# nirvanesque/headCT_foundation

Hardware: AMD Instinct MI355X
Metric: CT-volumes/sec MAE pretrain step (96^3, ViT-B/16^3, mask 0.75) (higher is better)
Workload: dtype bf16; 1 GPU; BASELINE config #2: MAE ViT-B/16^3, 96^3x1ch, mask 0.75, full train step (fwd+bwd+clip+AdamW+LR); per_gpu_batch=256, global_batch=256, parallelism=dp1, init=reference init, seed 42

## Files before the change

headct_foundation_amd/_lib.py:

```python
from __future__ import annotations

import ctypes as C
import os
from typing import Optional

HERE = os.path.dirname(os.path.abspath(__file__))
LIB_PATH = os.path.join(HERE, "libheadct_hip.so")

HCT_F32, HCT_BF16, HCT_F16 = 0, 1, 2
NORM_LAYERNORM, NORM_RMSNORM = 0, 1
HCT_ACT_NONE, HCT_ACT_GELU, HCT_ACT_DGELU, HCT_ACT_TANH, HCT_ACT_GELU_D, HCT_ACT_MULAUX = 0, 1, 2, 3, 4, 5
ACT_NONE, ACT_GELU, ACT_DGELU = 0, 1, 2

c_void_p, c_int, c_float, c_size_t, c_int64 = C.c_void_p, C.c_int, C.c_float, C.c_size_t, C.c_int64


class GemmArgs(C.Structure):
    _fields_ = [
        ("M", c_int), ("N", c_int), ("K", c_int),
        ("A", c_void_p), ("a_dtype", c_int), ("lda", c_int64), ("transA", c_int),
        ("B", c_void_p), ("b_dtype", c_int), ("ldb", c_int64), ("transB", c_int),
        ("C", c_void_p), ("c_dtype", c_int), ("ldc", c_int64),
        ("bias", c_void_p), ("residual", c_void_p), ("ldr", c_int64),
        ("act", c_int),
# ... 4 lines not shown


class GemmPlanInfo(C.Structure):
    _fields_ = [("kernel", c_int), ("epilogue_mode", c_int), ("fuse_colsum", c_int), ("row_tiles_per_wave", c_int), ("tiles", c_int),
                ("grid", c_int), ("sk_tiles", c_int), ("sk_wgs", c_int), ("splits", c_int), ("r_chunk", c_int), ("colsum_bytes", c_size_t),
                ("stream_k_offset", c_size_t), ("slab_bytes", c_size_t), ("workspace_bytes", c_size_t), ("walk_width", c_int)]


class ProfShape(C.Structure):
    _fields_ = [("M", c_int), ("N", c_int), ("K", c_int), ("mode", c_int), ("tiles", c_int), ("sk_tiles", c_int),
                ("launches", c_int64), ("total_ms", C.c_double), ("work", C.c_double), ("bytes", C.c_double)]


def prof_shapes(lib, kernel_class: int, cap: int = 256):
    buf = (ProfShape * cap)()
    n = lib.hct_prof_shapes(kernel_class, C.cast(buf, c_void_p), cap)
    if n < 0:
        raise HctError("hct_prof_shapes failed")
    return [buf[i] for i in range(min(n, cap))]


class MaeConfig(C.Structure):
    _fields_ = [
        ("input_size", c_int), ("patch_size", c_int), ("in_chans", c_int), ("mask_ratio", C.c_double),
        ("pos_embed", c_int),
        ("encoder_depth", c_int), ("encoder_embed_dim", c_int), ("encoder_mlp_dim", c_int), ("encoder_num_heads", c_int),
        ("decoder_depth", c_int), ("decoder_embed_dim", c_int), ("decoder_mlp_dim", c_int), ("decoder_num_heads", c_int),
        ("norm_pix_loss", c_int), ("use_bias", c_int),
        ("encoder_only", c_int), ("num_register_tokens", c_int), ("final_norm_eps", c_float),
        ("lora_rank", c_int),
        ("norm_kind", c_int),
        ("dropout_rate", c_float),
        ("drop_path_rate", c_float),
        ("patch_dropout", C.c_double),
    ]


class ParamInfo(C.Structure):
    _fields_ = [
        ("name", C.c_char * 96), ("ndim", c_int), ("shape", c_int64 * 5), ("offset", c_int64), ("numel", c_int64),
        ("requires_grad", c_int), ("is_matrix", c_int), ("bf16_t_offset", c_int64),
    ]


_PROTOS = {
    "hct_last_error_string": (C.c_char_p, []),
    "hct_version": (c_int, []),
    "hct_has_mfma_kernels": (c_int, []),
    "hct_gemm_workspace_bytes": (c_size_t, [C.POINTER(GemmArgs)]),
    "hct_gemm_nt_flags_offset": (c_size_t, [c_size_t]),
    "hct_gemm_describe": (c_int, [C.POINTER(GemmArgs), c_int, c_size_t, C.POINTER(GemmPlanInfo)]),
    "hct_gemm_stream_k_items": (c_int, [c_int, c_int, c_int, c_int, C.POINTER(C.c_uint32), C.POINTER(C.c_uint32)]),
    "hct_gemm_nt_walk": (c_int, [c_int, c_int, c_int, c_int, C.POINTER(c_int)]),
    "hct_set_cu_reserve": (None, [c_int]),
    "hct_gemm": (c_int, [C.POINTER(GemmArgs), c_void_p, c_size_t, c_void_p]),
    "hct_mask_rank": (c_int, [c_void_p, c_int, c_int, c_int, c_void_p, c_void_p, c_void_p, c_void_p]),
    "hct_patch_gather": (c_int, [c_void_p, c_int, c_void_p, c_int, c_int, c_int, c_int, c_int, c_int, c_void_p, c_int, c_void_p]),
    "hct_encoder_assemble_fwd": (c_int, [c_void_p, c_int, c_void_p, c_void_p, c_void_p, c_int, c_int, c_int, c_int, c_void_p, c_void_p]),
    "hct_encoder_assemble_bwd": (c_int, [c_void_p, c_void_p, c_int, c_int, c_int, c_int, c_void_p, c_int, c_void_p, c_void_p, c_void_p, c_size_t, c_void_p]),
    "hct_assemble_bwd_workspace_bytes": (c_size_t, [c_int]),
    "hct_layernorm_fwd": (c_int, [c_void_p, c_void_p, c_void_p, c_int, c_int, c_float, c_void_p, c_int, c_void_p, c_void_p, c_void_p]),
    "hct_layernorm_bwd_workspace_bytes": (c_size_t, [c_int, c_int]),
    "hct_layernorm_bwd": (c_int, [c_void_p, c_int, c_void_p, c_void_p, c_void_p, c_void_p, c_void_p, c_int, c_int, c_void_p, c_void_p,
                                  c_int, c_void_p, c_void_p, c_void_p, c_void_p, c_size_t, c_void_p]),
    "hct_layernorm_bwd_mapped": (c_int, [c_void_p, c_int, c_void_p, c_void_p, c_void_p, c_void_p, c_void_p, c_void_p, c_int, c_int, c_void_p,
                                         c_void_p, c_int, c_void_p, c_void_p, c_void_p, c_void_p, c_size_t, c_void_p]),
    "hct_rmsnorm_fwd": (c_int, [c_void_p, c_void_p, c_int, c_int, c_float, c_void_p, c_int, c_void_p, c_void_p]),
    "hct_rmsnorm_bwd_workspace_bytes": (c_size_t, [c_int, c_int]),
    "hct_rmsnorm_bwd": (c_int, [c_void_p, c_int, c_void_p, c_void_p, c_void_p, c_void_p, c_int, c_int, c_void_p, c_void_p, c_int, c_void_p,
                                c_void_p, c_void_p, c_size_t, c_void_p]),
    "hct_rmsnorm_bwd_mapped": (c_int, [c_void_p, c_int, c_void_p, c_void_p, c_void_p, c_void_p, c_void_p, c_int, c_int, c_void_p, c_void_p,
                                       c_int, c_void_p, c_void_p, c_void_p, c_size_t, c_void_p]),
    "hct_tail_rows": (c_int, [c_void_p, c_int, c_int, c_int, c_void_p, c_void_p, c_void_p]),
    "hct_gather_rows": (c_int, [c_void_p, c_void_p, c_int, c_int, c_void_p, c_void_p]),
    "hct_attention_fwd": (c_int, [c_void_p, c_int, c_int, c_int, c_int, c_int, c_void_p, c_void_p, c_void_p]),
    "hct_attention_bwd": (c_int, [c_void_p, c_void_p, c_void_p, c_void_p, c_int, c_int, c_int, c_int, c_int, c_void_p, c_void_p]),
    "hct_debug_force_simple_attention": (None, [c_int]),
    "hct_dropout_mask": (c_int, [C.c_uint64, c_int, c_int, c_int64, c_int, c_int, c_float, c_void_p, c_void_p]),
    "hct_dropout_apply": (c_int, [c_void_p, c_int, c_void_p, c_int, c_void_p, c_void_p, c_void_p, c_int64, c_int64, c_int64, c_int64, C.c_uint64,
                                  c_int, c_float, c_void_p]),
    "hct_attention_dropout_fwd": (c_int, [c_void_p, c_int, c_int, c_int, c_int, c_int, c_float, C.c_uint64, c_int, c_void_p, c_void_p, c_void_p]),
    "hct_attention_dropout_bwd": (c_int, [c_void_p, c_void_p, c_void_p, c_void_p, c_int, c_int, c_int, c_int, c_int, c_float, C.c_uint64, c_int,
                                          c_void_p, c_void_p]),
    "hct_drop_path_scales": (c_int, [C.c_uint64, C.POINTER(c_int), C.POINTER(c_float), c_int, c_int, c_void_p, c_void_p]),
    "hct_residual_drop_apply": (c_int, [c_void_p, c_int, c_void_p, c_int, c_void_p, c_int64, c_int64, c_void_p, C.c_uint64, c_int, c_float,
                                        c_void_p]),
    "hct_mae_plan_set_dropout": (c_int, [c_void_p, c_int, C.c_uint64]),
    "hct_decoder_assemble_fwd": (c_int, [c_void_p, c_int, c_void_p, c_void_p, c_void_p, c_void_p, c_int, c_int, c_int, c_int, c_void_p, c_void_p]),
    "hct_decoder_assemble_bwd": (c_int, [c_void_p, c_void_p, c_void_p, c_int, c_int, c_int, c_int, c_void_p, c_int, c_void_p, c_void_p,
                                         c_void_p, c_size_t, c_void_p]),
    "hct_masked_mse": (c_int, [c_void_p, c_int, c_void_p, c_int, c_void_p, c_int, c_int, c_int, c_int, c_int, c_float, c_void_p, c_void_p, c_void_p, c_void_p, c_void_p]),
    "hct_unpatchify": (c_int, [c_void_p, c_int, c_int, c_int, c_int, c_int, c_int, c_void_p, c_void_p]),
    "hct_vit_assemble_fwd": (c_int, [c_void_p, c_int, c_void_p, c_void_p, c_void_p, c_int, c_int, c_int, c_int, c_void_p, c_void_p]),
    "hct_channel_norm": (c_int, [c_void_p, c_void_p, c_void_p, c_float, c_void_p, c_int, c_int64, c_int, c_void_p]),
    "hct_query_attention": (c_int, [c_void_p, c_int, c_void_p, c_int, c_int, c_int, c_int, c_int, c_float, c_void_p, c_void_p]),
    "hct_head_linear": (c_int, [c_void_p, c_int64, c_int, c_void_p, c_void_p, c_float, c_void_p, c_void_p, c_int, c_void_p, c_int, c_int,
                                c_int, c_void_p]),
    "hct_batchnorm_stats": (c_int, [c_void_p, c_int, c_int, c_float, c_void_p, c_void_p, c_void_p, c_void_p, c_void_p]),
    "hct_softmax_xent": (c_int, [c_void_p, c_void_p, c_int, c_int, c_void_p, c_void_p, c_void_p, c_void_p]),
    "hct_sigmoid_bce_workspace_bytes": (c_size_t, [c_int, c_int]),
    "hct_sigmoid_bce": (c_int, [c_void_p, c_void_p, c_void_p, c_int, c_int, c_void_p, c_void_p, c_void_p, c_void_p, c_void_p, c_size_t, c_void_p]),
    "hct_mix_volumes": (c_int, [c_void_p, c_int, c_int, c_int, c_void_p, c_void_p, c_void_p]),
    "hct_mix_xent": (c_int, [c_void_p, c_void_p, c_void_p, c_float, c_int, c_int, c_void_p, c_void_p, c_void_p, c_void_p]),
    "hct_head_linear_wgrad": (c_int, [c_void_p, c_void_p, c_void_p, c_float, c_void_p, c_int, c_int, c_int, c_void_p, c_void_p, c_void_p]),
    "hct_bn_rows_workspace_bytes": (c_size_t, [c_int, c_int]),
    "hct_bn_stats_rows": (c_int, [c_void_p, c_int, c_int64, c_int, c_int, c_float, c_void_p, c_void_p, c_void_p, c_void_p, c_void_p,
# ... 207 lines not shown
```

headct_foundation_amd/csrc/gemm.hip:

```cpp
#include "common.h"
#include "gemm_plan.h"
#include "prof.h"

#include <cstdlib>
#include <cstring>
#include <vector>

namespace hct {

struct Epilogue {
  const float* bias;
  const float* residual;
  int64_t ldr;
  int act;
  void* aux; int aux_dtype; int64_t ldaux;
  void* C; int c_dtype; int64_t ldc;
  void* C2; int c2_dtype; int64_t ldc2;
  float alpha;
  float* colsum_partial;
  int aux_deriv;
};

__device__ __forceinline__ void store4(void* base, int dtype, int64_t off, f32x4 v) {
  if (dtype == HCT_BF16) Vec4<bf16>::store((bf16*)base + off, v);
// ... 218 lines not shown
    const int c = wave * 4 + i;
    const int row = c * 8 + (lane >> 3);
    const int src_chunk = (lane & 7) ^ ((row >> 1) & 7);
    voa[i] = (uint32_t)(row * lda * 2 + src_chunk * 16);
    vob[i] = (uint32_t)(row * ldb * 2 + src_chunk * 16);
  }
  auto stage = [&](int buf, int k0) {
    unsigned char* base = smem + buf * 32768;
#pragma unroll
    for (int i = 0; i < 4; ++i) {
      const int c = wave * 4 + i;
      __builtin_amdgcn_raw_ptr_buffer_load_lds(ra, (lds_void*)(base + c * 1024), 16, voa[i] + k0 * 2, 0, 0, 0);
      __builtin_amdgcn_raw_ptr_buffer_load_lds(rb, (lds_void*)(base + 16384 + c * 1024), 16, vob[i] + k0 * 2, 0, 0, 0);
    }
  };

  const int wr = wave >> 1, wc = wave & 1;
  const int frow = lane & 15, fchk = lane >> 4, swz = (lane >> 1) & 7;
  f32x4 acc[4][4];
#pragma unroll
  for (int i = 0; i < 4; ++i)
#pragma unroll
    for (int j = 0; j < 4; ++j) acc[i][j] = f32x4{0, 0, 0, 0};

  const int nk = K >> 6;
  stage(0, 0);
  __syncthreads();
  for (int kt = 0; kt < nk; ++kt) {
    const int buf = kt & 1;
    if (kt + 1 < nk) stage(buf ^ 1, (kt + 1) << 6);
    const unsigned char* sa = smem + buf * 32768 + (wr * 64 + frow) * 128;
    const unsigned char* sb = smem + buf * 32768 + 16384 + (wc * 64 + frow) * 128;
#pragma unroll
    for (int ks = 0; ks < 2; ++ks) {
      const int off = ((ks * 4 + fchk) ^ swz) << 4;
      bf16x8 af[4], bfr[4];
#pragma unroll
      for (int i = 0; i < 4; ++i) af[i] = *reinterpret_cast<const bf16x8*>(sa + i * 2048 + off);
#pragma unroll
      for (int j = 0; j < 4; ++j) bfr[j] = *reinterpret_cast<const bf16x8*>(sb + j * 2048 + off);
#pragma unroll
      for (int i = 0; i < 4; ++i)
#pragma unroll
        for (int j = 0; j < 4; ++j) acc[i][j] = __builtin_amdgcn_mfma_f32_16x16x32_bf16(bfr[j], af[i], acc[i][j], 0, 0, 0);
    }
    __syncthreads();
  }
#pragma unroll
  for (int i = 0; i < 4; ++i) {
    epilogue_tile16x64(e, smem + wave * kStageBytes, lane, m0 + wr * 64 + i * 16, n0 + wc * 64, M, N, acc[i]);
  }
}

__device__ __forceinline__ int swz64(int r) { return (0x1230 >> (((r >> 2) & 3) * 4)) & 3; }

__device__ __forceinline__ void epilogue_tile16x64_swz(const Epilogue& e, unsigned char* patch, int lane, int m_base, int n_base,
                                                       int M, int N, const f32x4* acc) {
  const int frow = lane & 15, fchk = lane >> 4;
#pragma unroll
  for (int j = 0; j < 4; ++j) *reinterpret_cast<f32x4*>(patch + frow * 256 + (((j * 4 + fchk) ^ frow) << 4)) = acc[j];
  const int rr = lane >> 4, cc = lane & 15;
  const int n = n_base + cc * 4;
  f32x4 v[4], r[4], u[4];
#pragma unroll
  for (int it = 0; it < 4; ++it) {
    const int row = it * 4 + rr;
    v[it] = *reinterpret_cast<const f32x4*>(patch + row * 256 + ((cc ^ row) << 4));
  }
  const bool nok = n < N;
  f32x4 bv = (e.bias && nok) ? Vec4<float>::load(e.bias + n) : f32x4{0, 0, 0, 0};
#pragma unroll
  for (int it = 0; it < 4; ++it) {
    const int m = m_base + it * 4 + rr;
    const bool ok = nok && m < M;
    r[it] = (e.residual && ok) ? Vec4<float>::load(e.residual + (int64_t)m * e.ldr + n) : f32x4{0, 0, 0, 0};
    u[it] = (e.act == HCT_ACT_DGELU && ok) ? load4(e.aux, e.aux_dtype, (int64_t)m * e.ldaux + n) : f32x4{0, 0, 0, 0};
  }
#pragma unroll
  for (int it = 0; it < 4; ++it) {
    const int m = m_base + it * 4 + rr;
    if (!(nok && m < M)) continue;
    f32x4 x = v[it] * e.alpha + bv;
    if (e.act == HCT_ACT_GELU) {
      if (e.aux) {
        f32x4 sv = x;
        if (e.aux_deriv) {
#pragma unroll
          for (int i = 0; i < 4; ++i) sv[i] = dgelu_erf(x[i]);
        }
        store4(e.aux, e.aux_dtype, (int64_t)m * e.ldaux + n, sv);
      }
#pragma unroll
      for (int i = 0; i < 4; ++i) x[i] = gelu_erf(x[i]);
    } else if (e.act == HCT_ACT_DGELU) {
#pragma unroll
      for (int i = 0; i < 4; ++i) x[i] *= e.aux_deriv ? u[it][i] : dgelu_erf(u[it][i]);
    }
    x += r[it];
    store4(e.C, e.c_dtype, (int64_t)m * e.ldc + n, x);
    if (e.C2) store4(e.C2, e.c2_dtype, (int64_t)m * e.ldc2 + n, x);
  }
}

__device__ __forceinline__ void epilogue_tile16x128(const Epilogue& e, unsigned char* patch, int lane, int m_base, int n_base,
                                                    int M, int N, const f32x4* acc) {
  const int frow = lane & 15, fchk = lane >> 4;
#pragma unroll
// ... 337 lines not shown


__device__ __forceinline__ i32x4 make_srd(const void* base, uint32_t num_records) {
  const uint64_t pa = (uint64_t)base;
  return i32x4{(int)__builtin_amdgcn_readfirstlane((uint32_t)pa), (int)(__builtin_amdgcn_readfirstlane((uint32_t)(pa >> 32)) & 0xFFFF),
               (int)__builtin_amdgcn_readfirstlane(num_records), 0x00020000};
}

__device__ __forceinline__ void dma16s(i32x4 rsrc, uint32_t lds_base, uint32_t voff, uint32_t soff) {
  asm volatile("s_mov_b32 m0, %0\n\ts_nop 0\n\tbuffer_load_dwordx4 %1, %2, %3 offen lds" ::"s"(lds_base), "v"(voff), "s"(rsrc), "s"(soff)
               : "memory", "m0");
}
__device__ __forceinline__ void dma16(i32x4 rsrc, uint32_t lds_base, uint32_t voff) {
  asm volatile("s_mov_b32 m0, %0\n\ts_nop 0\n\tbuffer_load_dwordx4 %1, %2, 0 offen lds" ::"s"(lds_base), "v"(voff), "s"(rsrc) : "memory", "m0");
}

#ifdef HCT_STAMPS
__device__ uint32_t* g_stamp_ptr = nullptr;
__device__ uint32_t g_stamp_words = 0;
#define HCT_STAMP(k)                                                                                   \
  do {                                                                                                 \
    unsigned long long t_;                                                                             \
    __builtin_amdgcn_sched_barrier(0);                                                                 \
    asm volatile("s_memrealtime %0\n\ts_waitcnt lgkmcnt(0)" : "=s"(t_)::"memory");                     \
    __builtin_amdgcn_sched_barrier(0);                                                                 \
    stamps = lane == ((tile_i * 4 + (k)) & 63) ? (uint32_t)t_ : stamps;                                \
  } while (0)
#define HCT_WAIT_BEGIN()                                                                               \
  unsigned long long w0_, w1_;                                                                         \
  __builtin_amdgcn_sched_barrier(0);                                                                   \
  asm volatile("s_memrealtime %0\n\ts_waitcnt lgkmcnt(0)" : "=s"(w0_)::"memory");                      \
  __builtin_amdgcn_sched_barrier(0)
#define HCT_WAIT_END()                                                                                 \
  __builtin_amdgcn_sched_barrier(0);                                                                   \
  asm volatile("s_memrealtime %0\n\ts_waitcnt lgkmcnt(0)" : "=s"(w1_)::"memory");                      \
  __builtin_amdgcn_sched_barrier(0);                                                                   \
  wait_acc += (uint32_t)(w1_ - w0_)
#else
#define HCT_STAMP(k)
#define HCT_WAIT_BEGIN()
#define HCT_WAIT_END()
#endif

constexpr int kSkErrWord = 512;

__device__ __forceinline__ unsigned sk_pub(unsigned seq_arg) { return ((seq_arg >> 31) ? seq_arg + 1u : seq_arg) & 0x0FFFFFFFu; }

__device__ __forceinline__ uint32_t xcc_id() {
  uint32_t v;
  asm volatile("s_getreg_b32 %0, hwreg(HW_REG_XCC_ID)" : "=s"(v));
  return v & 15;
}

template <int MODE, bool SK = false, int MT = 4>
__global__ void __launch_bounds__(512, 2) gemm_bf16_nt256_kernel(int M, int N, int K, const bf16* __restrict__ A, int64_t lda,
                                                                 const bf16* __restrict__ B, int64_t ldb, Epilogue e, int ntiles, int sk_tiles, int sk_wgs, unsigned char* __restrict__ sk_ws, unsigned sk_seq, int walk_w) {
  __shared__ __attribute__((aligned(16))) unsigned char smem[163840];
  constexpr int kBRing = 6 * 16384;
  static_assert(MT == 4 || (MT == 3 && !SK && (MODE == EPI_PLAIN_BF16 || MODE == EPI_RES_F32)), "192-row tiles: whole tiles, plain / +residual epilogues");
  const int lane = threadIdx.x & 63, wave = __builtin_amdgcn_readfirstlane(threadIdx.x >> 6);
  const int ntn = (N + 255) >> 8;
  float* const colsum_out = e.colsum_partial;

  constexpr int NP = 2;
  uint32_t voa[NP], vob[NP];
#pragma unroll
  for (int i = 0; i < NP; ++i) {
    const int row = ((wave & 7) * NP + i) * 16 + (lane >> 2);
    const int src_chunk = (lane & 3) ^ swz64(row);
    voa[i] = (uint32_t)(row * lda * 2 + src_chunk * 16);
    vob[i] = (uint32_t)(row * ldb * 2 + src_chunk * 16);
  }
  const int wm = wave >> 1, wn = wave & 1;
  const int frow = lane & 15, fchk = lane >> 4;
  const int foff = frow * 64 + ((fchk ^ swz64(frow)) << 4);
  const int nk = K >> 5;

  i32x4 ra, rb;
  const uint32_t lds0 = (uint32_t)(size_t)((__attribute__((address_space(3))) unsigned char*)smem);
  int m0 = 0, n0 = 0;
  auto set_tile_id = [&](int id, int s0) {
    const int tm = id / ntn, tn = id - tm * ntn;
    m0 = tm * (64 * MT);
    n0 = tn << 8;
    const bf16* Ab = A + (int64_t)m0 * lda + s0 * 32;
    const bf16* Bb = B + (int64_t)n0 * ldb + s0 * 32;
    ra = make_srd(Ab, clamp_records(((int64_t)(M - m0 - 1) * lda + K - s0 * 32) * 2));
    rb = make_srd(Bb, clamp_records(((int64_t)(N - n0 - 1) * ldb + K - s0 * 32) * 2));
  };
  auto dp_id = [&](int vb) { return nt_walk_id(nt_xcd_pos(vb, ntiles - sk_tiles), ntiles, ntn, sk_tiles, walk_w); };
  auto stage_a = [&](int t) {
    const uint32_t s0 = lds0 + (t % 6) * 16384;
    const uint32_t kb = (uint32_t)t * 64;
#pragma unroll
    for (int i = 0; i < NP; ++i) {
      const int c = wave * NP + i;
      if (MT == 4 || c < 4 * MT) {
        dma16s(ra, s0 + c * 1024, voa[i], kb);
        dma16s(ra, s0 + 16384 + c * 1024, voa[i], kb + 64);
      }
    }
  };
  auto stage_b = [&](int t) {
    const uint32_t s0 = lds0 + kBRing + (t & 3) * 16384;
    const uint32_t kb = (uint32_t)t * 64;
#pragma unroll
    for (int i = 0; i < NP; ++i) {
      const int c = wave * NP + i;
      dma16s(rb, s0 + c * 1024, vob[i], kb);
      dma16s(rb, s0 + 16384 + c * 1024, vob[i], kb + 64);
    }
  };
  f32x4 acc[MT][8];
  bf16x8 b_lo[4], b_hi[4], a0[MT], a1[MT];
  auto rd_a = [&](int t, bf16x8* af) {
    const unsigned char* sa = smem + (t % 6) * 16384 + wm * (16 * MT * 64) + foff;
#pragma unroll
    for (int i = 0; i < MT; ++i) af[i] = *reinterpret_cast<const bf16x8*>(sa + i * 1024);
  };
  auto rd_b = [&](int t, int half, bf16x8* bq) {
    const unsigned char* sb = smem + kBRing + (t & 3) * 16384 + wn * (128 * 64) + half * 4096 + foff;
#pragma unroll
    for (int j = 0; j < 4; ++j) bq[j] = *reinterpret_cast<const bf16x8*>(sb + j * 1024);
  };
  auto mma = [&](int half, const bf16x8* af, const bf16x8* bq) {
#pragma unroll
    for (int i = 0; i < MT; ++i)
#pragma unroll
      for (int j = 0; j < 4; ++j)
        acc[i][half * 4 + j] = __builtin_amdgcn_mfma_f32_16x16x32_bf16(bq[j], af[i], acc[i][half * 4 + j], 0, 0, 0);
  };
#ifdef HCT_STAMPS
  uint32_t stamps = 0, waits = 0, wait_acc = 0;
  int tile_i = 0;
#endif
  auto land_steady = [&]() {
    HCT_WAIT_BEGIN();
    if (MT == 3 && wave >= 6) asm volatile("s_waitcnt vmcnt(0) lgkmcnt(0)" ::: "memory");
    else asm volatile("s_waitcnt vmcnt(4) lgkmcnt(0)" ::: "memory");
    __builtin_amdgcn_s_barrier();
    HCT_WAIT_END();
  };
  auto land_all = [&]() {
    HCT_WAIT_BEGIN();
    asm volatile("s_waitcnt vmcnt(0)" ::: "memory");
    __builtin_amdgcn_s_barrier();
    HCT_WAIT_END();
  };
  auto land_top = [&](bool third) {
    if ((MT == 3 && wave >= 6) || !third) asm volatile("s_waitcnt vmcnt(4)" ::: "memory");
    else asm volatile("s_waitcnt vmcnt(8)" ::: "memory");
    __builtin_amdgcn_s_barrier();
  };
  auto stage_first = [&]() {
    stage_a(0);
    stage_b(0);
    stage_a(2);
  };
  const int P = nk >> 1;
  uint32_t it_first = 0, it_owner = 0;
  if (SK) stream_k_items(blockIdx.x, sk_tiles, sk_wgs, P, it_first, it_owner);
  int vb = blockIdx.x;
  uint32_t cit = 0;
  auto take_item = [&](uint32_t it) {
    set_tile_id((int)(it & 255), (int)((it >> 8) & 1023) * 2);
    cit = it;
  };
  auto next_item = [&]() -> bool {
    if (SK && it_owner) {
      take_item(it_owner);
      it_owner = 0;
      return true;
    }
    if (vb < ntiles - sk_tiles) {
      set_tile_id(dp_id(vb), 0);
      cit = (uint32_t)P << 18;
// ... 894 lines not shown
  for (int i = 0; i < n; ++i) {
    if (check)
      if (int rc = tn_group_check(jobs + i, i)) return rc;
    tj[i] = tn_group_job<bf16>(jobs + i, tile0);
    tile0 += tj[i].ntiles;
  }
  segs = tn_group_segments(tj);
  if ((int)segs.size() > tn_group_seg_capacity(n)) {
    set_error("hct_gemm_tn_group: %zu tile segments exceed the workspace's table (%d)", segs.size(), tn_group_seg_capacity(n));
    return HCT_E_WORKSPACE;
  }
  return 0;
}

}

using namespace hct;

extern "C" {

void hct_set_cu_reserve(int n) { g_cu_reserve = n < 0 ? 0 : n; }
void hct_debug_set_gemm_variant(int v) {
  if (v == -8 || v == -9) { g_tuning.sk_drop = v == -8; return; }
  if (v == -14 || v == -15) { g_tuning.mt3 = v == -14; return; }
  if (v <= -1000) { g_tuning.sk_min_k = -v - 1000; return; }
  if (v <= -20 && v >= -99) { g_tuning.walk_width = -v - 20; return; }
  if (v <= -100) { g_tuning.sk_gain_pairs = -v - 100; return; }
  g_tuning.nt_variant = v;
}
#ifdef HCT_STAMPS
int hct_debug_set_stamp_buffer(void* p, unsigned int n_words) {
  if (int rc = hct::check_hip(hipMemcpyToSymbol(HIP_SYMBOL(hct::g_stamp_words), &n_words, sizeof(n_words)), "stamp buffer size")) return rc;
  return hct::check_hip(hipMemcpyToSymbol(HIP_SYMBOL(hct::g_stamp_ptr), &p, sizeof(p)), "stamp buffer");
}
#endif

int hct_gemm_describe(const hct_gemm_args* a, int cus, size_t workspace_bytes, hct_gemm_plan_info* out) {
  HCT_REQUIRE(a && out && a->M >= 0 && a->N >= 0 && a->K >= 0, "hct_gemm_describe: bad arguments");
  *out = plan_gemm(a, cus > 0 ? cus : num_cus(), g_tuning, workspace_bytes);
  return 0;
}
int hct_gemm_stream_k_items(int grid, int sk_tiles, int sk_wgs, int pairs, uint32_t* first, uint32_t* owner) {
  HCT_REQUIRE(grid >= 0 && sk_tiles >= 0 && sk_wgs >= 0 && pairs > 0 && first && owner, "hct_gemm_stream_k_items: bad arguments");
  for (int wg = 0; wg < grid; ++wg) stream_k_items((unsigned)wg, sk_tiles, sk_wgs, pairs, first[wg], owner[wg]);
  return 0;
}

int hct_gemm_nt_walk(int tiles, int n_col_tiles, int sk_tiles, int walk_width, int* ids) {
  HCT_REQUIRE(tiles >= 0 && n_col_tiles > 0 && tiles % n_col_tiles == 0 && sk_tiles >= 0 && sk_tiles <= tiles && ids, "hct_gemm_nt_walk: bad arguments");
  for (int vb = 0; vb < tiles - sk_tiles; ++vb) ids[vb] = nt_walk_id(nt_xcd_pos(vb, tiles - sk_tiles), tiles, n_col_tiles, sk_tiles, walk_width);
  return 0;
}

size_t hct_gemm_workspace_bytes(const hct_gemm_args* a) { return plan_gemm(a, num_cus(), g_tuning, kUnlimited).workspace_bytes; }
size_t hct_gemm_nt_stream_k_bytes(void) { return kSkBytes; }
size_t hct_gemm_nt_flags_offset(size_t workspace_bytes) { return ws_layout(0, workspace_bytes).stream_k_offset; }

size_t hct_gemm_tn_group_workspace_bytes(int n_jobs) { return n_jobs > 0 ? tn_group_table_bytes(n_jobs) + tn_group_seg_bytes(n_jobs) + kTnSkBytes : 0; }

int hct_gemm_tn_group_prepare(const hct_gemm_args* jobs, int n, void* workspace, size_t workspace_bytes, void* stream) {
  HCT_REQUIRE(jobs && n > 0 && n <= 4096 && workspace, "hct_gemm_tn_group_prepare: bad arguments");
  if (workspace_bytes < hct_gemm_tn_group_workspace_bytes(n) || ((uintptr_t)workspace % 256) != 0) {
    set_error("hct_gemm_tn_group: workspace too small or not 256-byte aligned (%zu < %zu)", workspace_bytes, hct_gemm_tn_group_workspace_bytes(n));
    return HCT_E_WORKSPACE;
  }
  hipStream_t s = (hipStream_t)stream;
  std::vector<TnJob> tj;
  std::vector<TnSeg> segs;
  if (int rc = tn_group_build(jobs, n, true, tj, segs)) return rc;
  for (int first = 0; first < n; first += kTnGroupChunk) {
    TnJobChunk c;
    memset(&c, 0, sizeof(c));
    const int cnt = std::min(kTnGroupChunk, n - first);
    for (int i = 0; i < cnt; ++i) c.j[i] = tj[first + i];
    hipLaunchKernelGGL(tn_group_table_kernel, dim3(1), dim3(64), 0, s, (TnJob*)workspace, c, first, cnt);
  }
  TnSeg* dsegs = (TnSeg*)((unsigned char*)workspace + tn_group_table_bytes(n));
  for (int first = 0; first < (int)segs.size(); first += kTnSegChunk) {
    TnSegChunk c;
    memset(&c, 0, sizeof(c));
    const int cnt = std::min(kTnSegChunk, (int)segs.size() - first);
    for (int i = 0; i < cnt; ++i) c.s[i] = segs[first + i];
    hipLaunchKernelGGL(tn_group_seg_kernel, dim3(1), dim3(256), 0, s, dsegs, c, first, cnt);
  }
  if (int rc = check_hip(hipMemsetAsync((unsigned char*)workspace + tn_group_table_bytes(n) + tn_group_seg_bytes(n), 0, kTnSkHeadBytes, s),
                         "hct_gemm_tn_group: flag reset"))
    return rc;
  HCT_CHECK_LAUNCH("hct_gemm_tn_group_prepare");
  return 0;
}

int hct_gemm_tn_group_run(const hct_gemm_args* jobs, int n, void* workspace, size_t workspace_bytes, void* stream) {
  HCT_REQUIRE(jobs && n > 0 && workspace && workspace_bytes >= hct_gemm_tn_group_workspace_bytes(n), "hct_gemm_tn_group_run: bad arguments");
  hipStream_t s = (hipStream_t)stream;
  const int G = std::min(num_cus(), kSkMaxWgs);
  std::vector<TnJob> tj;
  std::vector<TnSeg> segs;
  if (int rc = tn_group_build(jobs, n, false, tj, segs)) return rc;
  int T = 0;
  double flops = 0, bytes = 0;
  for (int i = 0; i < n; ++i) {
    T += tj[i].ntiles;
    flops += 2.0 * jobs[i].M * jobs[i].N * jobs[i].K;
    bytes += 2.0 * jobs[i].K * (jobs[i].M + jobs[i].N) + 4.0 * jobs[i].M * jobs[i].N;
  }
  const int F = T / G, Rm = T - F * G;
// ... 48 lines not shown
```

headct_foundation_amd/csrc/gemm_plan.h:

```cpp
#pragma once
#include <stddef.h>
#include <stdint.h>
#include <string.h>

#include <algorithm>
#include <vector>

#include "../../include/headct_hip.h"

#ifdef __HIPCC__
#define HCT_HOST_DEVICE __host__ __device__ inline __attribute__((always_inline))
#else
#define HCT_HOST_DEVICE inline
#endif

namespace hct {

enum { EPI_GENERIC = 0, EPI_PLAIN_BF16 = 1, EPI_RES_F32 = 2, EPI_GELU_BF16 = 3, EPI_DGELU_BF16 = 4, EPI_PLAIN_F32 = 5,
       EPI_DGELU_CS = 6  };

constexpr int kSkMaxWgs = 256;
constexpr size_t kSkHeadBytes = 4096, kSkSlabBytes = 262144;
constexpr size_t kSkBytes = kSkHeadBytes + (size_t)kSkMaxWgs * kSkSlabBytes;
constexpr int kTnMaxFollowers = 1024;
// ... 74 lines not shown
      if (c >= wx) return nx * P;
      const int v = (int)(((int64_t)c * nx * P) / wx);
      const int r = v % P;
      return r == 1 ? v - 1 : (r == P - 1 ? v + 1 : v);
    };
    int b = sk_bound(j);
    const int en = sk_bound(j + 1);
    int t = b / P;
    const int off = b - t * P;
    if (off) {
      const int pe = en < (t + 1) * P ? en : (t + 1) * P;
      first = (uint32_t)(t0 + t) | ((uint32_t)off << 8) | ((uint32_t)(pe - b) << 18);
      b = pe;
      ++t;
    }
    if (b < en) {
      const int tend = (t + 1) * P;
      uint32_t nf = 0;
      for (int c2 = j + 1; c2 < wx && sk_bound(c2) < tend; ++c2) ++nf;
      owner = (uint32_t)(t0 + t) | ((uint32_t)((en < tend ? en : tend) - b) << 18) | (nf << 28) | 0x80000000u;
    }
    if (!first) { first = owner; owner = 0; }
  }
}

constexpr size_t kXcdL2Bytes = 4u << 20;
constexpr size_t kWalkWeightBudget = kXcdL2Bytes / 2;
constexpr int kXcdWindow = 32;

inline int nt_walk_width(int ntn, int K, int tiles, int G) {
  if (tiles <= G || ntn < 2) return ntn;
  const size_t panel = (size_t)256 * K * 2;
  const int wmax = (int)std::min<size_t>(kWalkWeightBudget / panel, kXcdWindow);
  if (wmax >= ntn || wmax < 2) return ntn;
  const int bands = ceil_div(ntn, wmax);
  return ceil_div(ntn, bands);
}

HCT_HOST_DEVICE int nt_xcd_pos(int vb, int nwg) {
  const int xcd = vb & 7, q = nwg >> 3, r = nwg & 7;
  return (xcd < r ? xcd * (q + 1) : r * (q + 1) + (xcd - r) * q) + (vb >> 3);
}

HCT_HOST_DEVICE int nt_walk_id(int pos, int ntiles, int ntn, int sk_tiles, int w) {
  if (w <= 0 || w >= ntn) return sk_tiles + pos;
  const int r0 = (sk_tiles + ntn - 1) / ntn;
  const int lead = (r0 * ntn < ntiles ? r0 * ntn : ntiles) - sk_tiles;
  if (pos < lead) return sk_tiles + pos;
  const int p = pos - lead, band = (ntiles / ntn - r0) * w;
  const int b = p / band, r = p - b * band;
  const int wb = ntn - b * w < w ? ntn - b * w : w;
  const int tr = r / wb;
  return (r0 + tr) * ntn + b * w + (r - tr * wb);
}

inline bool tn256_ok(const hct_gemm_args* a, const GemmTuning& t) {
  return t.nt_variant != 128 && a->c_dtype == HCT_F32 && !a->C2 && a->ldc % 4 == 0 && a->ldc * 256 < (1ll << 28) &&
         a->lda * 2 * 64 < (1ll << 31) && a->ldb * 2 * 64 < (1ll << 31);
}

inline void tn256_split(const hct_gemm_args* a, int G, int& splits, int& r_chunk) {
  const int tiles = std::max(1, ceil_div(a->M, 256) * ceil_div(a->N, 256));
  int s = std::max(1, G / tiles);
  int per = (a->K + s - 1) / s;
  per = std::max(128, (per + 63) / 64 * 64);
  while ((int64_t)per * std::max(a->lda, a->ldb) * 2 >= (1ll << 31)) per = std::max(128, per / 2 / 64 * 64);
  r_chunk = per;
  splits = (a->K + per - 1) / per;
}

inline void tn_split(const hct_gemm_args* a, int& splits, int& r_chunk) {
  const int tiles = std::max(1, ceil_div(a->M, 128) * ceil_div(a->N, 128));
  const int steps = (a->K + 63) / 64;
  int s = (1024 + tiles - 1) / tiles;
  if (s > steps / 4) s = steps / 4;
  if (s < 1) s = 1;
  int per = (steps + s - 1) / s;
  r_chunk = per * 64;
  splits = (a->K + r_chunk - 1) / r_chunk;
}

inline int colsum_chunks(int rows, int cols) {
  const int colblk = (cols + 255) / 256;
  int chunks = (1024 + colblk - 1) / colblk;
  if (chunks > (rows + 15) / 16) chunks = (rows + 15) / 16;
  return chunks < 1 ? 1 : chunks;
}
inline size_t colsum_ws(const hct_gemm_args* a) {
  if (!a->colsum_out) return 0;
  const size_t fused = (size_t)ceil_div(a->M, 256) * 4 * a->N * sizeof(float);
  return std::max(fused, (size_t)colsum_chunks(a->M, a->N) * a->N * sizeof(float));
}

struct WsLayout { size_t head_bytes, stream_k_offset; };
inline WsLayout ws_layout(size_t colsum_bytes, size_t workspace_bytes) {
  if (workspace_bytes < align256(colsum_bytes) + kSkBytes) return WsLayout{workspace_bytes, kNoOffset};
  const size_t off = (workspace_bytes - kSkBytes) & ~(size_t)255;
  return WsLayout{off, off};
}

inline GemmPlan plan_gemm(const hct_gemm_args* a, int num_cus, const GemmTuning& t, size_t available) {
  GemmPlan p;
  memset(&p, 0, sizeof(p));
  p.row_tiles_per_wave = 4;
  p.splits = 1;
  p.stream_k_offset = kNoOffset;
// ... 166 lines not shown
```

include/headct_hip.h:

```cpp
#ifndef HEADCT_HIP_H
#define HEADCT_HIP_H

#include <stddef.h>
#include <stdint.h>

#ifdef __cplusplus
extern "C" {
#endif

#define HCT_F32 0
#define HCT_BF16 1
#define HCT_F16 2

#define HCT_E_BADARG (-1)
#define HCT_E_UNSUPPORTED (-2)
#define HCT_E_WORKSPACE (-3)
#define HCT_E_STATE (-4)

#define HCT_ACT_NONE 0
#define HCT_ACT_GELU 1
#define HCT_ACT_DGELU 2
#define HCT_ACT_TANH 3
#define HCT_ACT_GELU_D 4
#define HCT_ACT_MULAUX 5

const char* hct_last_error_string(void);
int hct_version(void);
int hct_has_mfma_kernels(void);

typedef struct hct_gemm_args {
  int M, N, K;
  const void* A; int a_dtype; int64_t lda; int transA;
  const void* B; int b_dtype; int64_t ldb; int transB;
  void* C; int c_dtype; int64_t ldc;
  const float* bias;
  const float* residual;
  int64_t ldr;
  int act;
  void* aux; int aux_dtype; int64_t ldaux;
  void* C2; int c2_dtype; int64_t ldc2;
  float alpha;
  int force_generic;
  float* colsum_out;
  int workspace_armed;
} hct_gemm_args;

size_t hct_gemm_workspace_bytes(const hct_gemm_args* a);
size_t hct_gemm_nt_flags_offset(size_t workspace_bytes);
size_t hct_gemm_nt_stream_k_bytes(void);
void hct_set_cu_reserve(int n);
int hct_gemm(const hct_gemm_args* a, void* workspace, size_t workspace_bytes, void* stream);
#define HCT_GEMM_GENERIC 0
#define HCT_GEMM_NT128 1
#define HCT_GEMM_NT256 2
#define HCT_GEMM_TN128 3
#define HCT_GEMM_TN256 4
typedef struct hct_gemm_plan_info {
  int kernel;
  int epilogue_mode;
  int fuse_colsum;
  int row_tiles_per_wave;
  int tiles, grid;
  int sk_tiles, sk_wgs;
  int splits, r_chunk;
  size_t colsum_bytes;
  size_t stream_k_offset;
  size_t slab_bytes;
  size_t workspace_bytes;
  int walk_width;
} hct_gemm_plan_info;
int hct_gemm_describe(const hct_gemm_args* a, int num_cus, size_t workspace_bytes, hct_gemm_plan_info* out);
int hct_gemm_stream_k_items(int grid, int sk_tiles, int sk_wgs, int pairs, uint32_t* first, uint32_t* owner);
int hct_gemm_nt_walk(int tiles, int n_col_tiles, int sk_tiles, int walk_width, int* ids);
size_t hct_gemm_tn_group_workspace_bytes(int n_jobs);
int hct_gemm_tn_group_prepare(const hct_gemm_args* jobs, int n_jobs, void* workspace, size_t workspace_bytes, void* stream);
int hct_gemm_tn_group_run(const hct_gemm_args* jobs, int n_jobs, void* workspace, size_t workspace_bytes, void* stream);

int hct_mask_rank(const float* noise, int B, int L, int K, int32_t* ids_restore, int32_t* ids_shuffle,
                  float* mask, void* stream);

int hct_patch_gather(const void* x, int x_dtype , const int32_t* ids_shuffle, int B, int C, int S, int P, int L, int K,
                     void* rows, int rows_dtype, void* stream);

int hct_encoder_assemble_fwd(const void* tok, int tok_dtype, const float* cls, const float* pos,
                             const int32_t* ids_shuffle, int B, int L, int K, int D, float* h0, void* stream);
int hct_encoder_assemble_bwd(const float* dh0, const int32_t* ids_restore, int B, int L, int K, int D,
                             void* dtok, int dtok_dtype, float* dcls, float* dpos, void* workspace,
                             size_t workspace_bytes, void* stream);
size_t hct_assemble_bwd_workspace_bytes(int D);

int hct_layernorm_fwd(const float* x, const float* gamma, const float* beta, int rows, int D, float eps,
                      void* y, int y_dtype, float* mean, float* rstd, void* stream);
size_t hct_layernorm_bwd_workspace_bytes(int rows, int D);
int hct_layernorm_bwd(const void* dy, int dy_dtype, const float* x, const float* mean, const float* rstd,
                      const float* gamma, const float* dres, int rows, int D, float* dx, void* dx_shadow,
                      int shadow_dtype, float* dgamma, float* dbeta, float* dcolsum, void* workspace,
                      size_t workspace_bytes, void* stream);
int hct_layernorm_bwd_mapped(const void* dy, int dy_dtype, const float* x, const float* mean, const float* rstd,
                             const float* gamma, const float* dres, const int32_t* dres_rows, int rows, int D, float* dx,
                             void* dx_shadow, int shadow_dtype, float* dgamma, float* dbeta, float* dcolsum, void* workspace,
                             size_t workspace_bytes, void* stream);
int hct_rmsnorm_fwd(const float* x, const float* gamma, int rows, int D, float eps, void* y, int y_dtype, float* rstd,
                    void* stream);
size_t hct_rmsnorm_bwd_workspace_bytes(int rows, int D);
int hct_rmsnorm_bwd(const void* dy, int dy_dtype, const float* x, const float* rstd, const float* gamma, const float* dres,
                    int rows, int D, float* dx, void* dx_shadow, int shadow_dtype, float* dgamma, float* dcolsum,
                    void* workspace, size_t workspace_bytes, void* stream);
int hct_rmsnorm_bwd_mapped(const void* dy, int dy_dtype, const float* x, const float* rstd, const float* gamma,
                           const float* dres, const int32_t* dres_rows, int rows, int D, float* dx, void* dx_shadow,
                           int shadow_dtype, float* dgamma, float* dcolsum, void* workspace, size_t workspace_bytes,
                           void* stream);
int hct_tail_rows(const int32_t* ids_restore, int B, int L, int K, int32_t* tail_rows, int32_t* tail_inv, void* stream);
int hct_gather_rows(const void* src, const int32_t* idx, int n_rows, int row_bytes, void* dst, void* stream);

int hct_attention_fwd(const void* qkv, int B, int N, int H, int dh, int dtype, void* o, float* lse, void* stream);
int hct_attention_bwd(const void* qkv, const void* o, const void* d_o, const float* lse, int B, int N, int H,
                      int dh, int dtype, void* dqkv, void* stream);

int hct_dropout_mask(uint64_t seed, int site, int kind, int64_t n, int BH, int N, float p, unsigned char* out, void* stream);
int hct_dropout_apply(const void* x, int x_dtype, void* y, int y_dtype, const float* residual, const void* x2, void* y2,
                      int64_t batches, int64_t stride, int64_t off, int64_t seg, uint64_t seed, int site, float p, void* stream);
int hct_attention_dropout_fwd(const void* qkv, int B, int N, int H, int dh, int dtype, float p, uint64_t seed, int site, void* o,
                              float* lse, void* stream);
int hct_attention_dropout_bwd(const void* qkv, const void* o, const void* d_o, const float* lse, int B, int N, int H, int dh,
                              int dtype, float p, uint64_t seed, int site, void* dqkv, void* stream);
int hct_drop_path_scales(uint64_t seed, const int* sites, const float* rates, int n_sites, int B, float* out, void* stream);
// ... 257 lines not shown
```

Measured before the change: 7228 CT-volumes/s.

## Repack NT256 GEMM LDS staging into 128-byte paired-kstep lines with new swizzle

Changes the shared-memory layout of the NT 256x256 bf16 GEMM so that two consecutive 32-wide k-steps share one 128-byte row line, using a new XOR swizzle. The DMA now issues two 8-row pieces per wave from base and +16-row descriptors, and fragment reads index by k-step parity within a pair. The goal is wider, more contiguous global reads and fewer LDS bank conflicts. It adds a host-side line-map export and compile-time checks of the offsets, and risks stage-ring mismatches since buffers are now indexed in pairs.

New measurement: 7249 CT-volumes/s (median of 6 runs). Within noise of the previous version (+0.3%).

```diff
diff --git a/headct_foundation_amd/_lib.py b/headct_foundation_amd/_lib.py
--- a/headct_foundation_amd/_lib.py
+++ b/headct_foundation_amd/_lib.py
@@ -80,6 +80,7 @@
     "hct_gemm_describe": (c_int, [C.POINTER(GemmArgs), c_int, c_size_t, C.POINTER(GemmPlanInfo)]),
     "hct_gemm_stream_k_items": (c_int, [c_int, c_int, c_int, c_int, C.POINTER(C.c_uint32), C.POINTER(C.c_uint32)]),
     "hct_gemm_nt_walk": (c_int, [c_int, c_int, c_int, c_int, C.POINTER(c_int)]),
+    "hct_gemm_nt_line_map": (c_int, [c_int, C.POINTER(c_int), C.POINTER(c_int), C.POINTER(c_int), C.POINTER(c_int)]),
     "hct_set_cu_reserve": (None, [c_int]),
     "hct_gemm": (c_int, [C.POINTER(GemmArgs), c_void_p, c_size_t, c_void_p]),
     "hct_mask_rank": (c_int, [c_void_p, c_int, c_int, c_int, c_void_p, c_void_p, c_void_p, c_void_p]),
diff --git a/headct_foundation_amd/csrc/gemm.hip b/headct_foundation_amd/csrc/gemm.hip
--- a/headct_foundation_amd/csrc/gemm.hip
+++ b/headct_foundation_amd/csrc/gemm.hip
@@ -294,7 +294,6 @@
   }
 }
 
-__device__ __forceinline__ int swz64(int r) { return (0x1230 >> (((r >> 2) & 3) * 4)) & 3; }
 
 __device__ __forceinline__ void epilogue_tile16x64_swz(const Epilogue& e, unsigned char* patch, int lane, int m_base, int n_base,
                                                        int M, int N, const f32x4* acc) {
@@ -738,6 +737,20 @@
   return v & 15;
 }
 
+constexpr bool nt_rd_split_ok(int mt) {
+  for (int w = 0; w < 8; ++w)
+    for (int l = 0; l < 64; ++l)
+      for (int ks = 0; ks < 2; ++ks) {
+        const int f = nt_frag_off(l & 15, 0, l >> 4) ^ (ks << 6);
+        for (int i = 0; i < mt; ++i)
+          if (nt_rd_a_off(mt, w, l, i, ks) != (w >> 1) * (16 * mt * 128) + f + i * 2048) return false;
+        for (int h = 0; h < 2; ++h)
+          for (int j = 0; j < 4; ++j)
+            if (nt_rd_b_off(w, l, h, j, ks) != (w & 1) * (128 * 128) + h * 8192 + f + j * 2048) return false;
+      }
+  return true;
+}
+
 template <int MODE, bool SK = false, int MT = 4>
 __global__ void __launch_bounds__(512, 2) gemm_bf16_nt256_kernel(int M, int N, int K, const bf16* __restrict__ A, int64_t lda,
                                                                  const bf16* __restrict__ B, int64_t ldb, Epilogue e, int ntiles, int sk_tiles, int sk_wgs, unsigned char* __restrict__ sk_ws, unsigned sk_seq, int walk_w) {
@@ -749,20 +762,20 @@
   float* const colsum_out = e.colsum_partial;
 
   constexpr int NP = 2;
+  static_assert(nt_pair_dma_dst(2, 5).row == nt_pair_dma_dst(0, 5).row + 16 && nt_pair_dma_dst(2, 5).chunk == nt_pair_dma_dst(0, 5).chunk, "");
   uint32_t voa[NP], vob[NP];
 #pragma unroll
   for (int i = 0; i < NP; ++i) {
-    const int row = ((wave & 7) * NP + i) * 16 + (lane >> 2);
-    const int src_chunk = (lane & 3) ^ swz64(row);
-    voa[i] = (uint32_t)(row * lda * 2 + src_chunk * 16);
-    vob[i] = (uint32_t)(row * ldb * 2 + src_chunk * 16);
+    const NtDmaDst d = nt_pair_dma_dst(nt_wave_piece(wave & 7, i), lane);
+    voa[i] = (uint32_t)(d.row * lda * 2 + d.chunk * 16);
+    vob[i] = (uint32_t)(d.row * ldb * 2 + d.chunk * 16);
   }
   const int wm = wave >> 1, wn = wave & 1;
   const int frow = lane & 15, fchk = lane >> 4;
-  const int foff = frow * 64 + ((fchk ^ swz64(frow)) << 4);
+  const int foff = nt_frag_off(frow, 0, fchk);
   const int nk = K >> 5;
 
-  i32x4 ra, rb;
+  i32x4 ra, rb, ra16, rb16;
   const uint32_t lds0 = (uint32_t)(size_t)((__attribute__((address_space(3))) unsigned char*)smem);
   int m0 = 0, n0 = 0;
   auto set_tile_id = [&](int id, int s0) {
@@ -773,6 +786,8 @@
     const bf16* Bb = B + (int64_t)n0 * ldb + s0 * 32;
     ra = make_srd(Ab, clamp_records(((int64_t)(M - m0 - 1) * lda + K - s0 * 32) * 2));
     rb = make_srd(Bb, clamp_records(((int64_t)(N - n0 - 1) * ldb + K - s0 * 32) * 2));
+    ra16 = make_srd(Ab + 16 * lda, clamp_records(((int64_t)(M - m0 - 17) * lda + K - s0 * 32) * 2));
+    rb16 = make_srd(Bb + 16 * ldb, clamp_records(((int64_t)(N - n0 - 17) * ldb + K - s0 * 32) * 2));
   };
   auto dp_id = [&](int vb) { return nt_walk_id(nt_xcd_pos(vb, ntiles - sk_tiles), ntiles, ntn, sk_tiles, walk_w); };
   auto stage_a = [&](int t) {
@@ -780,10 +795,10 @@
     const uint32_t kb = (uint32_t)t * 64;
 #pragma unroll
     for (int i = 0; i < NP; ++i) {
-      const int c = wave * NP + i;
-      if (MT == 4 || c < 4 * MT) {
-        dma16s(ra, s0 + c * 1024, voa[i], kb);
-        dma16s(ra, s0 + 16384 + c * 1024, voa[i], kb + 64);
+      const int p = nt_wave_piece(wave, i);
+      if (MT == 4 || p < 8 * MT) {
+        dma16s(ra, s0 + p * 1024, voa[i], kb);
+        dma16s(ra16, s0 + (p + 2) * 1024, voa[i], kb);
       }
     }
   };
@@ -792,22 +807,23 @@
     const uint32_t kb = (uint32_t)t * 64;
 #pragma unroll
     for (int i = 0; i < NP; ++i) {
-      const int c = wave * NP + i;
-      dma16s(rb, s0 + c * 1024, vob[i], kb);
-      dma16s(rb, s0 + 16384 + c * 1024, vob[i], kb + 64);
+      const int p = nt_wave_piece(wave, i);
+      dma16s(rb, s0 + p * 1024, vob[i], kb);
+      dma16s(rb16, s0 + (p + 2) * 1024, vob[i], kb);
     }
   };
   f32x4 acc[MT][8];
   bf16x8 b_lo[4], b_hi[4], a0[MT], a1[MT];
+  static_assert(nt_rd_split_ok(MT), "fragment offsets");
   auto rd_a = [&](int t, bf16x8* af) {
-    const unsigned char* sa = smem + (t % 6) * 16384 + wm * (16 * MT * 64) + foff;
-#pragma unroll
-    for (int i = 0; i < MT; ++i) af[i] = *reinterpret_cast<const bf16x8*>(sa + i * 1024);
+    const unsigned char* sa = smem + ((t >> 1) % 3) * kNtPairBytes + wm * (16 * MT * 128) + (foff ^ ((t & 1) << 6));
+#pragma unroll
+    for (int i = 0; i < MT; ++i) af[i] = *reinterpret_cast<const bf16x8*>(sa + i * 2048);
   };
   auto rd_b = [&](int t, int half, bf16x8* bq) {
-    const unsigned char* sb = smem + kBRing + (t & 3) * 16384 + wn * (128 * 64) + half * 4096 + foff;
-#pragma unroll
-    for (int j = 0; j < 4; ++j) bq[j] = *reinterpret_cast<const bf16x8*>(sb + j * 1024);
+    const unsigned char* sb = smem + kBRing + ((t >> 1) & 1) * kNtPairBytes + wn * (128 * 128) + half * 8192 + (foff ^ ((t & 1) << 6));
+#pragma unroll
+    for (int j = 0; j < 4; ++j) bq[j] = *reinterpret_cast<const bf16x8*>(sb + j * 2048);
   };
   auto mma = [&](int half, const bf16x8* af, const bf16x8* bq) {
 #pragma unroll
@@ -1808,6 +1824,28 @@
   return 0;
 }
 
+int hct_gemm_nt_line_map(int mt, int* dma, int* issuer, int* rd_a, int* rd_b) {
+  HCT_REQUIRE((mt == 3 || mt == 4) && dma && issuer && rd_a && rd_b, "hct_gemm_nt_line_map: bad arguments");
+  for (int piece = 0; piece < 8 * mt; ++piece)
+    for (int lane = 0; lane < 64; ++lane) {
+      const NtDmaDst d = nt_pair_dma_dst(piece, lane);
+      int* o = dma + (piece * 64 + lane) * 3;
+      o[0] = d.lds_off; o[1] = d.row; o[2] = d.chunk;
+    }
+  for (int piece = 0; piece < 8 * mt; ++piece) issuer[piece] = -1;
+  for (int wave = 0; wave < 8; ++wave)
+    for (int i = 0; i < kNtPiecesPerWave; ++i)
+      if (nt_wave_piece(wave, i) < 8 * mt) issuer[nt_wave_piece(wave, i)] = wave;
+  for (int wave = 0; wave < 8; ++wave)
+    for (int lane = 0; lane < 64; ++lane)
+      for (int ks = 0; ks < 2; ++ks) {
+        for (int i = 0; i < mt; ++i) rd_a[((wave * 64 + lane) * mt + i) * 2 + ks] = nt_rd_a_off(mt, wave, lane, i, ks);
+        for (int h = 0; h < 2; ++h)
+          for (int j = 0; j < 4; ++j) rd_b[((wave * 64 + lane) * 8 + h * 4 + j) * 2 + ks] = nt_rd_b_off(wave, lane, h, j, ks);
+      }
+  return 0;
+}
+
 size_t hct_gemm_workspace_bytes(const hct_gemm_args* a) { return plan_gemm(a, num_cus(), g_tuning, kUnlimited).workspace_bytes; }
 size_t hct_gemm_nt_stream_k_bytes(void) { return kSkBytes; }
 size_t hct_gemm_nt_flags_offset(size_t workspace_bytes) { return ws_layout(0, workspace_bytes).stream_k_offset; }
diff --git a/headct_foundation_amd/csrc/gemm_plan.h b/headct_foundation_amd/csrc/gemm_plan.h
--- a/headct_foundation_amd/csrc/gemm_plan.h
+++ b/headct_foundation_amd/csrc/gemm_plan.h
@@ -150,6 +150,23 @@
   const int wb = ntn - b * w < w ? ntn - b * w : w;
   const int tr = r / wb;
   return (r0 + tr) * ntn + b * w + (r - tr * wb);
+}
+
+constexpr int kNtPairBytes = 32768, kNtPieceRows = 8, kNtPiecesPerWave = 4;
+struct NtDmaDst { int lds_off, row, chunk; };
+HCT_HOST_DEVICE constexpr int nt_line_swz(int row) { return (row >> 1) & 7; }
+HCT_HOST_DEVICE constexpr NtDmaDst nt_pair_dma_dst(int piece, int lane) {
+  return NtDmaDst{piece * 1024 + lane * 16, piece * kNtPieceRows + (lane >> 3), (lane & 7) ^ nt_line_swz(piece * kNtPieceRows + (lane >> 3))};
+}
+HCT_HOST_DEVICE constexpr int nt_frag_off(int row_in_tile, int kstep_in_pair, int fchk) {
+  return row_in_tile * 128 + (((kstep_in_pair * 4 + fchk) ^ nt_line_swz(row_in_tile)) << 4);
+}
+HCT_HOST_DEVICE constexpr int nt_wave_piece(int wave, int i) { return wave * kNtPiecesPerWave + i; }
+HCT_HOST_DEVICE constexpr int nt_rd_a_off(int mt, int wave, int lane, int i, int kstep_in_pair) {
+  return nt_frag_off((wave >> 1) * 16 * mt + i * 16 + (lane & 15), kstep_in_pair, lane >> 4);
+}
+HCT_HOST_DEVICE constexpr int nt_rd_b_off(int wave, int lane, int half, int j, int kstep_in_pair) {
+  return nt_frag_off((wave & 1) * 128 + half * 64 + j * 16 + (lane & 15), kstep_in_pair, lane >> 4);
 }
 
 inline bool tn256_ok(const hct_gemm_args* a, const GemmTuning& t) {
diff --git a/include/headct_hip.h b/include/headct_hip.h
--- a/include/headct_hip.h
+++ b/include/headct_hip.h
@@ -72,6 +72,7 @@
 int hct_gemm_describe(const hct_gemm_args* a, int num_cus, size_t workspace_bytes, hct_gemm_plan_info* out);
 int hct_gemm_stream_k_items(int grid, int sk_tiles, int sk_wgs, int pairs, uint32_t* first, uint32_t* owner);
 int hct_gemm_nt_walk(int tiles, int n_col_tiles, int sk_tiles, int walk_width, int* ids);
+int hct_gemm_nt_line_map(int row_tiles_per_wave, int* dma, int* issuer, int* rd_a, int* rd_b);
 size_t hct_gemm_tn_group_workspace_bytes(int n_jobs);
 int hct_gemm_tn_group_prepare(const hct_gemm_args* jobs, int n_jobs, void* workspace, size_t workspace_bytes, void* stream);
 int hct_gemm_tn_group_run(const hct_gemm_args* jobs, int n_jobs, void* workspace, size_t workspace_bytes, void* stream);
```
